# zjwfufu/FateAvatar

Hardware: AMD Instinct MI355X
Metric: render+backward frames/sec at 512^2, 100k Gaussians (higher is better)
Workload: dtype f32

## Files before the change

fateavatar_amd/csrc/fr_preprocess_bwd.hip:

```cpp
#include "fr_bind_math.hpp"

namespace fr {

__constant__ float bSH_C0 = 0.28209479177387814f;
__constant__ float bSH_C1 = 0.4886025119029199f;
__constant__ float bSH_C2[5] = {1.0925484305920792f, -1.0925484305920792f, 0.31539156525252005f,
                                -1.0925484305920792f, 0.5462742152960396f};
__constant__ float bSH_C3[7] = {-0.5900435899266435f, 2.890611442640554f, -0.4570457994644658f, 0.3731763325901154f,
                                -0.4570457994644658f, 1.445305721320277f,  -0.5900435899266435f};

struct PreBwdArgs {
    int P, D, M, W, H, raw;
    float tan_fovx, tan_fovy, focal_x, focal_y, scale_modifier;
    const float* means3D;
    const float* scales;
    const float* rotations;
    const float* shs;
    const float* cov3D_precomp;
    const float* view;
    const float* proj;
    const float* campos;
    const int* radii;
    GeomView g;
    fr_grads out;
    float* grad_accum;
    float* denom;
    float* overflow_out;
    const DeviceCounts* counts;
    uint32_t acc;
    int bound;
    BindArgs bind;
    BindGrads bg;
};

enum { G_MEANS2D = 0, G_COLORS, G_OPACITY, G_MEANS3D, G_COV3D, G_SH, G_SCALES, G_ROTATIONS };

__device__ __forceinline__ void put(float* p, float v, bool add) { *p = add ? *p + v : v; }

__device__ __forceinline__ void store3(float* p, size_t i, float a, float b, float c, bool add)
{
    if (!p) return;
    if (add) a += p[3 * i], b += p[3 * i + 1], c += p[3 * i + 2];
    p[3 * i] = a, p[3 * i + 1] = b, p[3 * i + 2] = c;
}

__host__ __device__ constexpr bool prebwd_rows_by16(int M3) { return M3 % 4 == 0 && M3 <= 48; }
__host__ __device__ constexpr int prebwd_row_stride(int M3)
{
    return prebwd_rows_by16(M3) ? (((M3 / 4) & 1) ? M3 : M3 + 4) : (M3 | 1);
}

struct PreBwdIn {
    int radius;
    float mean[3], q[4], sc[3], c3[6];
    float opacity;
    uint32_t cl;
    float dd[9];
    float4 r0, r1, r2;
    uint32_t overflow;
    float ga, dn;
    float old_m3[3], old_sc[3], old_q[4], old_op;
};

template <class T> using GlobalPtr = const __attribute__((address_space(1))) T*;
template <class T> __device__ __forceinline__ GlobalPtr<T> as_global(const T* p) { return (GlobalPtr<T>)p; }
typedef float PreBwdF4 __attribute__((ext_vector_type(4)));

__device__ __forceinline__ void preprocess_bwd_fetch(const PreBwdArgs& a, const int li, PreBwdIn& in)
{
    const size_t i = (size_t)li;
    const auto adds = [&](int k) { return ((a.acc >> k) & 1u) != 0u; };
    const int* radii_ = a.radii;
    const DeviceCounts* counts_ = a.counts;
    const float *accum_ = a.g.accum, *means3D_ = a.means3D, *scales_ = a.scales, *rotations_ = a.rotations, *cov3D_ = a.cov3D_precomp;
    const float *opacity_act_ = a.g.opacity_act, *dcolor_ddir_ = a.g.dcolor_ddir, *shs = a.shs;
    const uint8_t* clamped_ = a.g.clamped;
    const float *grad_accum_ = a.grad_accum, *denom_ = a.denom;
    asm volatile("" : "+s"(radii_), "+s"(counts_), "+s"(accum_), "+s"(means3D_), "+s"(scales_), "+s"(rotations_), "+s"(cov3D_),
                 "+s"(opacity_act_), "+s"(dcolor_ddir_), "+s"(shs), "+s"(clamped_), "+s"(grad_accum_), "+s"(denom_));
    const auto radii = as_global(radii_);
    const auto counts = as_global(counts_);
    const auto accum = as_global(accum_), means3D = as_global(means3D_), scales = as_global(scales_), rotations = as_global(rotations_);
    const auto cov3D = as_global(cov3D_), opacity_act = as_global(opacity_act_), dcolor_ddir = as_global(dcolor_ddir_);
    const auto clamped = as_global(clamped_);
    const auto grad_accum = as_global(grad_accum_), denom = as_global(denom_);
    in.radius = radii[li];
    in.overflow = counts->overflow;
    const GlobalPtr<PreBwdF4> row4 = (GlobalPtr<PreBwdF4>)(accum + i * kAccumStride);
    const PreBwdF4 r0 = row4[0], r1 = row4[1], r2 = row4[2];
    in.r0 = make_float4(r0.x, r0.y, r0.z, r0.w), in.r1 = make_float4(r1.x, r1.y, r1.z, r1.w), in.r2 = make_float4(r2.x, r2.y, r2.z, r2.w);
    for (int k = 0; k < 3; k++) in.mean[k] = means3D[3 * i + k];
    for (int k = 0; k < 4; k++) in.q[k] = 0.f;
    for (int k = 0; k < 3; k++) in.sc[k] = 0.f;
    for (int k = 0; k < 6; k++) in.c3[k] = 0.f;
    if (scales) {
        for (int k = 0; k < 4; k++) in.q[k] = rotations[4 * i + k];
        for (int k = 0; k < 3; k++) in.sc[k] = scales[3 * i + k];
    }
    if (cov3D)
        for (int k = 0; k < 6; k++) in.c3[k] = cov3D[6 * i + k];
    in.opacity = opacity_act[li];
    in.cl = 0u;
    for (int k = 0; k < 9; k++) in.dd[k] = 0.f;
    if (shs) {
        in.cl = clamped[li];
        for (int k = 0; k < 9; k++) in.dd[k] = dcolor_ddir[i * 9 + k];
    }
    in.ga = in.dn = 0.f;
    if (grad_accum) in.ga = grad_accum[i];
    if (denom) in.dn = denom[i];
    for (int k = 0; k < 3; k++) in.old_m3[k] = 0.f, in.old_sc[k] = 0.f;
    for (int k = 0; k < 4; k++) in.old_q[k] = 0.f;
    in.old_op = 0.f;
    if (a.acc) {
        if (adds(G_MEANS3D) && a.out.dL_dmeans3D)
            for (int k = 0; k < 3; k++) in.old_m3[k] = a.out.dL_dmeans3D[3 * i + k];
        if (adds(G_SCALES) && a.out.dL_dscales)
            for (int k = 0; k < 3; k++) in.old_sc[k] = a.out.dL_dscales[3 * i + k];
        if (adds(G_ROTATIONS) && a.out.dL_drotations)
            for (int k = 0; k < 4; k++) in.old_q[k] = a.out.dL_drotations[4 * i + k];
        if (adds(G_OPACITY) && a.out.dL_dopacity) in.old_op = a.out.dL_dopacity[i];
    }
}

template <bool PLANES>
__device__ __forceinline__ void preprocess_bwd_one(const PreBwdArgs& a, const CameraRegs& cam, const PreBwdIn& in,
                                                   const int idx, float* row, const bool by16)
{
    const size_t i = (size_t)idx;
    const int Mc = a.M;
    const int radius = in.radius;
    const auto adds = [&](int k) { return ((a.acc >> k) & 1u) != 0u; };
    if (!(radius > 0)) {
        if (row && by16) {
            float4* r4 = reinterpret_cast<float4*>(row);
            for (int k = 0; k < (Mc * 3) / 4; k++) r4[k] = make_float4(0.f, 0.f, 0.f, 0.f);
        } else if (row)
            for (int k = 0; k < Mc * 3; k++) row[k] = 0.f;
        if (!adds(G_MEANS2D)) store3(a.out.dL_dmeans2D, i, 0.f, 0.f, 0.f, false);
        if (!adds(G_COLORS)) store3(a.out.dL_dcolors, i, 0.f, 0.f, 0.f, false);
        if (a.out.dL_dopacity && !adds(G_OPACITY)) a.out.dL_dopacity[i] = 0.f;
        if (!adds(G_MEANS3D)) store3(a.out.dL_dmeans3D, i, 0.f, 0.f, 0.f, false);
        if (a.out.dL_dcov3D && !adds(G_COV3D))
            for (int k = 0; k < 6; k++) a.out.dL_dcov3D[6 * i + k] = 0.f;
        if (a.out.dL_dsh && !row && !adds(G_SH))
            for (int k = 0; k < Mc * 3; k++) a.out.dL_dsh[i * Mc * 3 + k] = 0.f;
        if (!adds(G_SCALES)) store3(a.out.dL_dscales, i, 0.f, 0.f, 0.f, false);
        if (a.out.dL_drotations && !adds(G_ROTATIONS))
            for (int k = 0; k < 4; k++) a.out.dL_drotations[4 * i + k] = 0.f;
        if (a.bound) bind_bwd_zero(idx, a.bg);
        return;
    }
    const float old_m3[3] = {in.old_m3[0], in.old_m3[1], in.old_m3[2]}, old_sc[3] = {in.old_sc[0], in.old_sc[1], in.old_sc[2]};
    const float old_q[4] = {in.old_q[0], in.old_q[1], in.old_q[2], in.old_q[3]}, old_op = in.old_op;
    float acc[12];
    {
        float4* row4 = reinterpret_cast<float4*>(a.g.accum + i * kAccumStride);
        const float4 r0 = in.r0, r1 = in.r1, r2 = in.r2;
        row4[0] = row4[1] = row4[2] = make_float4(0.f, 0.f, 0.f, 0.f);
        acc[0] = r0.x, acc[1] = r0.y, acc[2] = r0.z, acc[3] = r0.w, acc[4] = r1.x, acc[5] = r1.y, acc[6] = r1.z,
        acc[7] = r1.w, acc[8] = r2.x, acc[9] = r2.y, acc[10] = r2.z, acc[11] = r2.w;
    }
    const float3 mean = make_float3(in.mean[0], in.mean[1], in.mean[2]);
    const float* vm = cam.view;
    float q_r = 0.f, q_x = 0.f, q_y = 0.f, q_z = 0.f, rot_inv = 1.0f;
    float sc[3] = {0.f, 0.f, 0.f};
    float c3[6];
    if (a.scales) {
        q_r = in.q[0], q_x = in.q[1], q_y = in.q[2], q_z = in.q[3];
        sc[0] = in.sc[0], sc[1] = in.sc[1], sc[2] = in.sc[2];
        if (a.raw) {
            sc[0] = act_exp(sc[0]), sc[1] = act_exp(sc[1]), sc[2] = act_exp(sc[2]);
            rot_inv = act_rot_inv_norm(q_r, q_x, q_y, q_z);
            q_r *= rot_inv, q_x *= rot_inv, q_y *= rot_inv, q_z *= rot_inv;
        }
    }
    if (a.cov3D_precomp) {
        for (int k = 0; k < 6; k++) c3[k] = in.c3[k];
    } else {
        cov3d_from_scale_rot(sc[0], sc[1], sc[2], q_r, q_x, q_y, q_z, a.scale_modifier, c3);
    }

    float3 t = xform4x3(mean, vm);
    const float limx = 1.3f * a.tan_fovx, limy = 1.3f * a.tan_fovy;
    const float txtz = t.x / t.z, tytz = t.y / t.z;
    t.x = fminf(limx, fmaxf(-limx, txtz)) * t.z;
    t.y = fminf(limy, fmaxf(-limy, tytz)) * t.z;
    const float x_grad_mul = txtz < -limx || txtz > limx ? 0 : 1;
    const float y_grad_mul = tytz < -limy || tytz > limy ? 0 : 1;
    const float h_x = a.focal_x, h_y = a.focal_y;
    const float j00 = h_x / t.z, j02 = -(h_x * t.x) / (t.z * t.z);
    const float j11 = h_y / t.z, j12 = -(h_y * t.y) / (t.z * t.z);
    float T0[3], T1[3];
    for (int w = 0; w < 3; w++) {
        const float W0 = vm[4 * w], W1 = vm[4 * w + 1], W2 = vm[4 * w + 2];
        T0[w] = W0 * j00 + W1 * 0.0f + W2 * j02;
        T1[w] = W0 * 0.0f + W1 * j11 + W2 * j12;
    }
    const float V[3][3] = {{c3[0], c3[1], c3[2]}, {c3[1], c3[3], c3[4]}, {c3[2], c3[4], c3[5]}};
    float A0[3], A1[3];
    for (int c = 0; c < 3; c++) {
        A0[c] = T0[0] * V[0][c] + T0[1] * V[1][c] + T0[2] * V[2][c];
        A1[c] = T1[0] * V[0][c] + T1[1] * V[1][c] + T1[2] * V[2][c];
    }
    float ca = A0[0] * T0[0] + A0[1] * T0[1] + A0[2] * T0[2];
    const float cb = A1[0] * T0[0] + A1[1] * T0[1] + A1[2] * T0[2];
    float cc = A1[0] * T1[0] + A1[1] * T1[1] + A1[2] * T1[2];
    ca += 0.3f;
    cc += 0.3f;
    const float denom = ca * cc - cb * cb;
    const float det_inv = 1.f / denom;
    const float4 co = make_float4(cc * det_inv, -cb * det_inv, ca * det_inv, in.opacity);
    const float g2x = acc[ACC_MX] * (0.5f * a.W);
    const float g2y = acc[ACC_MY] * (0.5f * a.H);
    const float dcx = -0.5f * acc[ACC_CA], dcy = -0.5f * acc[ACC_CB], dcz = -0.5f * acc[ACC_CC];
    const float dop = (co.w != 0.f) ? acc[ACC_OP] / co.w : 0.f;
    float dcol[3] = {acc[ACC_R], acc[ACC_G], acc[ACC_B]};
    store3(a.out.dL_dmeans2D, i, g2x, g2y, 0.f, adds(G_MEANS2D));
    if (!in.overflow) {
        if (a.grad_accum) a.grad_accum[i] = in.ga + sqrtf(g2x * g2x + g2y * g2y);
        if (a.denom) a.denom[i] = in.dn + 1.0f;
    }
    store3(a.out.dL_dcolors, i, dcol[0], dcol[1], dcol[2], adds(G_COLORS));
    if (a.out.dL_dopacity) a.out.dL_dopacity[i] = old_op + (a.raw ? dop * co.w * (1.0f - co.w) : dop);

    float dL_da = 0, dL_db = 0, dL_dc = 0;
    const float denom2inv = 1.0f / ((denom * denom) + 0.0000001f);
    float dcov[6] = {0, 0, 0, 0, 0, 0};
    if (denom2inv != 0) {
        dL_da = denom2inv * (-cc * cc * dcx + 2 * cb * cc * dcy + (denom - ca * cc) * dcz);
        dL_dc = denom2inv * (-ca * ca * dcz + 2 * ca * cb * dcy + (denom - ca * cc) * dcx);
        dL_db = denom2inv * 2 * (cb * cc * dcx - (denom + 2 * cb * cb) * dcy + ca * cb * dcz);
        dcov[0] = (T0[0] * T0[0] * dL_da + T0[0] * T1[0] * dL_db + T1[0] * T1[0] * dL_dc);
        dcov[3] = (T0[1] * T0[1] * dL_da + T0[1] * T1[1] * dL_db + T1[1] * T1[1] * dL_dc);
        dcov[5] = (T0[2] * T0[2] * dL_da + T0[2] * T1[2] * dL_db + T1[2] * T1[2] * dL_dc);
        dcov[1] = 2 * T0[0] * T0[1] * dL_da + (T0[0] * T1[1] + T0[1] * T1[0]) * dL_db + 2 * T1[0] * T1[1] * dL_dc;
        dcov[2] = 2 * T0[0] * T0[2] * dL_da + (T0[0] * T1[2] + T0[2] * T1[0]) * dL_db + 2 * T1[0] * T1[2] * dL_dc;
        dcov[4] = 2 * T0[2] * T0[1] * dL_da + (T0[1] * T1[2] + T0[2] * T1[1]) * dL_db + 2 * T1[1] * T1[2] * dL_dc;
    }
    if (a.out.dL_dcov3D)
        for (int k = 0; k < 6; k++) put(a.out.dL_dcov3D + 6 * i + k, dcov[k], adds(G_COV3D));

    float dT0[3], dT1[3];
    for (int c = 0; c < 3; c++) {
        const float tv0 = T0[0] * V[c][0] + T0[1] * V[c][1] + T0[2] * V[c][2];
        const float tv1 = T1[0] * V[c][0] + T1[1] * V[c][1] + T1[2] * V[c][2];
        dT0[c] = 2 * tv0 * dL_da + tv1 * dL_db;
        dT1[c] = 2 * tv1 * dL_dc + tv0 * dL_db;
    }
    const float dL_dJ00 = vm[0] * dT0[0] + vm[4] * dT0[1] + vm[8] * dT0[2];
    const float dL_dJ02 = vm[2] * dT0[0] + vm[6] * dT0[1] + vm[10] * dT0[2];
    const float dL_dJ11 = vm[1] * dT1[0] + vm[5] * dT1[1] + vm[9] * dT1[2];
    const float dL_dJ12 = vm[2] * dT1[0] + vm[6] * dT1[1] + vm[10] * dT1[2];
    const float tz = 1.f / t.z, tz2 = tz * tz, tz3 = tz2 * tz;
    const float dL_dtx = x_grad_mul * -h_x * tz2 * dL_dJ02;
    const float dL_dty = y_grad_mul * -h_y * tz2 * dL_dJ12;
    const float dL_dtz = -h_x * tz2 * dL_dJ00 - h_y * tz2 * dL_dJ11 + (2 * h_x * t.x) * tz3 * dL_dJ02 + (2 * h_y * t.y) * tz3 * dL_dJ12;
    float dmx = vm[0] * dL_dtx + vm[1] * dL_dty + vm[2] * dL_dtz;
    float dmy = vm[4] * dL_dtx + vm[5] * dL_dty + vm[6] * dL_dtz;
    float dmz = vm[8] * dL_dtx + vm[9] * dL_dty + vm[10] * dL_dtz;

    {
        const float* proj = cam.proj;
        const float4 m_hom = xform4x4(mean, proj);
        const float m_w = 1.0f / (m_hom.w + 0.0000001f);
        const float mul1 = (proj[0] * mean.x + proj[4] * mean.y + proj[8] * mean.z + proj[12]) * m_w * m_w;
        const float mul2 = (proj[1] * mean.x + proj[5] * mean.y + proj[9] * mean.z + proj[13]) * m_w * m_w;
        const float px = (proj[0] * m_w - proj[3] * mul1) * g2x + (proj[1] * m_w - proj[3] * mul2) * g2y;
        const float py = (proj[4] * m_w - proj[7] * mul1) * g2x + (proj[5] * m_w - proj[7] * mul2) * g2y;
        const float pz = (proj[8] * m_w - proj[11] * mul1) * g2x + (proj[9] * m_w - proj[11] * mul2) * g2y;
        dmx += px, dmy += py, dmz += pz;
    }

    if (a.shs) {
        const float dox = mean.x - cam.campos[0], doy = mean.y - cam.campos[1], doz = mean.z - cam.campos[2];
        const float len = sqrtf(dox * dox + doy * doy + doz * doz);
        const float x = dox / len, y = doy / len, z = doz / len;
        const uint32_t cl = in.cl;
        float dRGB[3];
        for (int c = 0; c < 3; c++) dRGB[c] = dcol[c] * (((cl >> c) & 1) ? 0 : 1);
        const float* dd = in.dd;
        const float dRGBdx[3] = {dd[0], dd[1], dd[2]}, dRGBdy[3] = {dd[3], dd[4], dd[5]}, dRGBdz[3] = {dd[6], dd[7], dd[8]};
        const int deg = a.D;
        const int used = (deg + 1) * (deg + 1);
        auto write_row = [&](float* dsh, const bool dsh_adds) {
#define DSH(k, c, v_) put(dsh + (k) * 3 + (c), (v_), dsh_adds)
            for (int c = 0; c < 3; c++) {
                DSH(0, c, bSH_C0 * dRGB[c]);
                if (deg > 0) {
                    DSH(1, c, (-bSH_C1 * y) * dRGB[c]);
                    DSH(2, c, (bSH_C1 * z) * dRGB[c]);
                    DSH(3, c, (-bSH_C1 * x) * dRGB[c]);
                    if (deg > 1) {
                        const float xx = x * x, yy = y * y, zz = z * z;
                        const float xy = x * y, yz = y * z, xz = x * z;
                        DSH(4, c, (bSH_C2[0] * xy) * dRGB[c]);
                        DSH(5, c, (bSH_C2[1] * yz) * dRGB[c]);
                        DSH(6, c, (bSH_C2[2] * (2.f * zz - xx - yy)) * dRGB[c]);
                        DSH(7, c, (bSH_C2[3] * xz) * dRGB[c]);
                        DSH(8, c, (bSH_C2[4] * (xx - yy)) * dRGB[c]);
                        if (deg > 2) {
                            DSH(9, c, (bSH_C3[0] * y * (3.f * xx - yy)) * dRGB[c]);
                            DSH(10, c, (bSH_C3[1] * xy * z) * dRGB[c]);
                            DSH(11, c, (bSH_C3[2] * y * (4.f * zz - xx - yy)) * dRGB[c]);
                            DSH(12, c, (bSH_C3[3] * z * (2.f * zz - 3.f * xx - 3.f * yy)) * dRGB[c]);
                            DSH(13, c, (bSH_C3[4] * x * (4.f * zz - xx - yy)) * dRGB[c]);
                            DSH(14, c, (bSH_C3[5] * z * (xx - yy)) * dRGB[c]);
                            DSH(15, c, (bSH_C3[6] * x * (xx - 3.f * yy)) * dRGB[c]);
                        }
                    }
                }
            }
            if (!dsh_adds)
                for (int k = used; k < Mc; k++) dsh[k * 3] = 0.f, dsh[k * 3 + 1] = 0.f, dsh[k * 3 + 2] = 0.f;
#undef DSH
        };
        auto write_row_by16 = [&](float* dsh) {
            float f[16] = {0.f, 0.f, 0.f, 0.f, 0.f, 0.f, 0.f, 0.f, 0.f, 0.f, 0.f, 0.f, 0.f, 0.f, 0.f, 0.f};
            f[0] = bSH_C0;
            if (deg > 0) {
                f[1] = -bSH_C1 * y, f[2] = bSH_C1 * z, f[3] = -bSH_C1 * x;
                if (deg > 1) {
                    const float xx = x * x, yy = y * y, zz = z * z;
                    const float xy = x * y, yz = y * z, xz = x * z;
                    f[4] = bSH_C2[0] * xy, f[5] = bSH_C2[1] * yz, f[6] = bSH_C2[2] * (2.f * zz - xx - yy);
                    f[7] = bSH_C2[3] * xz, f[8] = bSH_C2[4] * (xx - yy);
                    if (deg > 2) {
                        f[9] = bSH_C3[0] * y * (3.f * xx - yy), f[10] = bSH_C3[1] * xy * z;
                        f[11] = bSH_C3[2] * y * (4.f * zz - xx - yy), f[12] = bSH_C3[3] * z * (2.f * zz - 3.f * xx - 3.f * yy);
                        f[13] = bSH_C3[4] * x * (4.f * zz - xx - yy), f[14] = bSH_C3[5] * z * (xx - yy);
                        f[15] = bSH_C3[6] * x * (xx - 3.f * yy);
                    }
                }
            }
            float4* d4 = reinterpret_cast<float4*>(dsh);
            const int pieces = (Mc * 3) / 4;
#pragma unroll
            for (int j = 0; j < 12; j++) {
                if (j >= pieces) break;
                float v[4];
#pragma unroll
                for (int t = 0; t < 4; t++) {
                    const int k = (4 * j + t) / 3, c = (4 * j + t) % 3;
                    v[t] = k < used ? f[k] * dRGB[c] : 0.f;
                }
                d4[j] = make_float4(v[0], v[1], v[2], v[3]);
            }
        };
        if (row && by16) write_row_by16(row);
        else if (row) write_row(row, false);
        else if (a.out.dL_dsh) write_row(a.out.dL_dsh + i * Mc * 3, adds(G_SH));
        const float ddx = dRGBdx[0] * dRGB[0] + dRGBdx[1] * dRGB[1] + dRGBdx[2] * dRGB[2];
        const float ddy = dRGBdy[0] * dRGB[0] + dRGBdy[1] * dRGB[1] + dRGBdy[2] * dRGB[2];
        const float ddz = dRGBdz[0] * dRGB[0] + dRGBdz[1] * dRGB[1] + dRGBdz[2] * dRGB[2];
        const float sum2 = dox * dox + doy * doy + doz * doz;
        const float invsum32 = 1.0f / sqrtf(sum2 * sum2 * sum2);
        dmx += ((+sum2 - dox * dox) * ddx - doy * dox * ddy - doz * dox * ddz) * invsum32;
        dmy += (-dox * doy * ddx + (sum2 - doy * doy) * ddy - doz * doy * ddz) * invsum32;
        dmz += (-dox * doz * ddx - doy * doz * ddy + (sum2 - doz * doz) * ddz) * invsum32;
    } else if (a.out.dL_dsh && !row && !adds(G_SH)) {
        for (int k = 0; k < Mc * 3; k++) a.out.dL_dsh[i * Mc * 3 + k] = 0.f;
    }
    if (PLANES) {
        const float dz = acc[ACC_Z];
        dmx += dz * vm[2], dmy += dz * vm[6], dmz += dz * vm[10];
    }
    store3(a.out.dL_dmeans3D, i, old_m3[0] + dmx, old_m3[1] + dmy, old_m3[2] + dmz, false);
    const float g_mean[3] = {dmx, dmy, dmz};
    float g_scl[3] = {0.f, 0.f, 0.f}, g_rot[4] = {0.f, 0.f, 0.f, 0.f};

    if (a.scales) {
        const float r = q_r, x = q_x, y = q_y, z = q_z;
        const float s[3] = {a.scale_modifier * sc[0], a.scale_modifier * sc[1], a.scale_modifier * sc[2]};
        const float Rc[3][3] = {{1.f - 2.f * (y * y + z * z), 2.f * (x * y - r * z), 2.f * (x * z + r * y)},
                                {2.f * (x * y + r * z), 1.f - 2.f * (x * x + z * z), 2.f * (y * z - r * x)},
                                {2.f * (x * z - r * y), 2.f * (y * z + r * x), 1.f - 2.f * (x * x + y * y)}};
        const float dS[3][3] = {{dcov[0], 0.5f * dcov[1], 0.5f * dcov[2]},
                                {0.5f * dcov[1], dcov[3], 0.5f * dcov[4]},
                                {0.5f * dcov[2], 0.5f * dcov[4], dcov[5]}};
        float dM[3][3];
        for (int c = 0; c < 3; c++)
            for (int w = 0; w < 3; w++)
                dM[c][w] = (s[w] * Rc[0][w] * 2.0f) * dS[c][0] + (s[w] * Rc[1][w] * 2.0f) * dS[c][1] + (s[w] * Rc[2][w] * 2.0f) * dS[c][2];
        float dMt[3][3];
        for (int c = 0; c < 3; c++)
            for (int w = 0; w < 3; w++) dMt[c][w] = dM[w][c];
        const float dsx = Rc[0][0] * dMt[0][0] + Rc[1][0] * dMt[0][1] + Rc[2][0] * dMt[0][2];
        const float dsy = Rc[0][1] * dMt[1][0] + Rc[1][1] * dMt[1][1] + Rc[2][1] * dMt[1][2];
        const float dsz = Rc[0][2] * dMt[2][0] + Rc[1][2] * dMt[2][1] + Rc[2][2] * dMt[2][2];
        g_scl[0] = a.raw ? dsx * sc[0] : dsx, g_scl[1] = a.raw ? dsy * sc[1] : dsy, g_scl[2] = a.raw ? dsz * sc[2] : dsz;
        store3(a.out.dL_dscales, i, old_sc[0] + g_scl[0], old_sc[1] + g_scl[1], old_sc[2] + g_scl[2], false);
        for (int w = 0; w < 3; w++) dMt[0][w] *= s[0], dMt[1][w] *= s[1], dMt[2][w] *= s[2];
#define Dm(c_, r_) dMt[c_][r_]
        if (a.out.dL_drotations || a.bound) {
            float dq[4];
            dq[0] = 2 * z * (Dm(0, 1) - Dm(1, 0)) + 2 * y * (Dm(2, 0) - Dm(0, 2)) + 2 * x * (Dm(1, 2) - Dm(2, 1));
            dq[1] = 2 * y * (Dm(1, 0) + Dm(0, 1)) + 2 * z * (Dm(2, 0) + Dm(0, 2)) + 2 * r * (Dm(1, 2) - Dm(2, 1)) - 4 * x * (Dm(2, 2) + Dm(1, 1));
            dq[2] = 2 * x * (Dm(1, 0) + Dm(0, 1)) + 2 * r * (Dm(2, 0) - Dm(0, 2)) + 2 * z * (Dm(1, 2) + Dm(2, 1)) - 4 * y * (Dm(2, 2) + Dm(0, 0));
            dq[3] = 2 * r * (Dm(0, 1) - Dm(1, 0)) + 2 * x * (Dm(2, 0) + Dm(0, 2)) + 2 * y * (Dm(1, 2) + Dm(2, 1)) - 4 * z * (Dm(1, 1) + Dm(0, 0));
            if (a.raw) {
                const float dot = r * dq[0] + x * dq[1] + y * dq[2] + z * dq[3];
                dq[0] = (dq[0] - r * dot) * rot_inv;
                dq[1] = (dq[1] - x * dot) * rot_inv;
                dq[2] = (dq[2] - y * dot) * rot_inv;
                dq[3] = (dq[3] - z * dot) * rot_inv;
            }
            if (a.out.dL_drotations)
                for (int k = 0; k < 4; k++) a.out.dL_drotations[4 * i + k] = old_q[k] + dq[k];
            for (int k = 0; k < 4; k++) g_rot[k] = dq[k];
        }
#undef Dm
    } else {
        if (!adds(G_SCALES)) store3(a.out.dL_dscales, i, 0.f, 0.f, 0.f, false);
        if (a.out.dL_drotations && !adds(G_ROTATIONS))
            for (int k = 0; k < 4; k++) a.out.dL_drotations[4 * i + k] = 0.f;
    }
    if (a.bound) bind_bwd(a.bind, idx, g_mean, g_rot, g_scl, a.bg);
}

template <bool ADD>
__device__ __forceinline__ void unstage_rows_t(float* __restrict__ dst, const float* src, int stride, int rows, int row_len, int lane)
{
    const int total = rows * row_len;
    const unsigned magic = (unsigned)((0x100000000ull + (unsigned)row_len - 1u) / (unsigned)row_len);
    constexpr int kBatch = ADD ? 6 : 1;
    for (int base = lane * 4; base < total; base += 64 * 4 * kBatch) {
        float4 o[kBatch];
        if (ADD) {
#pragma unroll
            for (int u = 0; u < kBatch; u++) {
                const int c = base + u * 64 * 4;
                o[u] = make_float4(0.f, 0.f, 0.f, 0.f);
                if (c + 3 < total) {
                    o[u] = *reinterpret_cast<const float4*>(dst + c);
                } else {
                    if (c < total) o[u].x = dst[c];
                    if (c + 1 < total) o[u].y = dst[c + 1];
                    if (c + 2 < total) o[u].z = dst[c + 2];
                }
            }
        }
#pragma unroll
        for (int u = 0; u < kBatch; u++) {
            const int c = base + u * 64 * 4;
            if (c >= total) break;
            float v[4];
#pragma unroll
            for (int k = 0; k < 4; k++) {
                const int e = c + k;
                const int r = (int)__umulhi((unsigned)e, magic);
                v[k] = (e < total) ? src[r * stride + (e - r * row_len)] : 0.f;
            }
            if (ADD) v[0] += o[u].x, v[1] += o[u].y, v[2] += o[u].z, v[3] += o[u].w;
            if (c + 3 < total) *reinterpret_cast<float4*>(dst + c) = make_float4(v[0], v[1], v[2], v[3]);
            else
                for (int k = 0; k < 4; k++)
                    if (c + k < total) dst[c + k] = v[k];
        }
    }
}
template <bool ADD>
__device__ __forceinline__ void unstage_rows_by16_t(float* __restrict__ dst, const float* src, int stride, int rows, int row_len, int lane)
{
    const int total = rows * row_len;
    const unsigned magic = (unsigned)((0x100000000ull + (unsigned)row_len - 1u) / (unsigned)row_len);
    constexpr int kBatch = ADD ? 6 : 1;
    for (int base = lane * 4; base < total; base += 64 * 4 * kBatch) {
        float4 o[kBatch];
        if (ADD) {
#pragma unroll
            for (int u = 0; u < kBatch; u++) {
                const int c = base + u * 64 * 4;
                o[u] = make_float4(0.f, 0.f, 0.f, 0.f);
                if (c < total) o[u] = *reinterpret_cast<const float4*>(dst + c);
            }
        }
#pragma unroll
        for (int u = 0; u < kBatch; u++) {
            const int c = base + u * 64 * 4;
            if (c >= total) break;
            const int r = (int)__umulhi((unsigned)c, magic);
            float4 v = *reinterpret_cast<const float4*>(src + r * stride + (c - r * row_len));
            if (ADD) v.x += o[u].x, v.y += o[u].y, v.z += o[u].z, v.w += o[u].w;
            *reinterpret_cast<float4*>(dst + c) = v;
        }
    }
}
__device__ __forceinline__ void unstage_rows(float* __restrict__ dst, const float* src, int stride, int rows, int row_len, int lane,
                                             bool add)
{
    if (prebwd_rows_by16(row_len)) {
        if (add) unstage_rows_by16_t<true>(dst, src, stride, rows, row_len, lane);
        else unstage_rows_by16_t<false>(dst, src, stride, rows, row_len, lane);
    } else {
        if (add) unstage_rows_t<true>(dst, src, stride, rows, row_len, lane);
        else unstage_rows_t<false>(dst, src, stride, rows, row_len, lane);
    }
}

#ifndef FR_PREBWD_WAVES
#define FR_PREBWD_WAVES 4
#endif
constexpr int kPreBwdWaves = FR_PREBWD_WAVES;

template <bool PLANES>
__device__ __forceinline__ void preprocess_bwd_body(const PreBwdArgs& a)
{
    extern __shared__ __attribute__((aligned(16))) float s_rows[];
    if ((int)(blockIdx.x * blockDim.x) >= a.P) return;
    const int idx = blockIdx.x * blockDim.x + threadIdx.x;
    const int lane = threadIdx.x & 63, wave = threadIdx.x >> 6;
    const int M3 = a.M * 3, stride = prebwd_row_stride(M3);
    const int wave_first = blockIdx.x * (64 * kPreBwdWaves) + wave * 64;
    const int rows = min(64, a.P - wave_first);
    const bool staged = a.shs != nullptr && a.out.dL_dsh != nullptr;
    float* w_rows = s_rows + (size_t)wave * 64 * stride;
    PreBwdIn in;
    preprocess_bwd_fetch(a, min(idx, a.P - 1), in);
    const float cam_x = camera_request(a.view, a.proj, a.campos, lane);
    asm volatile("" ::: "memory");
    const CameraRegs cam = camera_broadcast(cam_x);
    asm volatile("" : "+v"(in.cl), "+v"(in.ga), "+v"(in.dn), "+v"(in.opacity), "+v"(in.radius));
    if (a.overflow_out && blockIdx.x == 0 && threadIdx.x == 0) *a.overflow_out = in.overflow ? 1.0f : 0.0f;
    if (idx < a.P) preprocess_bwd_one<PLANES>(a, cam, in, idx, staged ? w_rows + lane * stride : nullptr, prebwd_rows_by16(M3));
    __syncthreads();
    if (staged && rows > 0) unstage_rows(a.out.dL_dsh + (size_t)wave_first * M3, w_rows, stride, rows, M3, lane, ((a.acc >> G_SH) & 1u) != 0u);
}

__global__ void __launch_bounds__(64 * kPreBwdWaves) k_preprocess_bwd(PreBwdArgs a) { preprocess_bwd_body<false>(a); }
__global__ void __launch_bounds__(64 * kPreBwdWaves) k_preprocess_bwd_batch(BatchOf<PreBwdArgs> b) { preprocess_bwd_body<false>(b.v[blockIdx.y]); }
__global__ void __launch_bounds__(64 * kPreBwdWaves) k_preprocess_bwd_planes(PreBwdArgs a) { preprocess_bwd_body<true>(a); }
__global__ void __launch_bounds__(64 * kPreBwdWaves) k_preprocess_bwd_planes_batch(BatchOf<PreBwdArgs> b) { preprocess_bwd_body<true>(b.v[blockIdx.y]); }

int launch_blend_backward(int n, const BackwardCall* calls, const GeomView* g, const ImageView* v, bool planes, hipStream_t s, bool debug);

int launch_backward(int n, const BackwardCall* calls, hipStream_t s)
{
    GeomView g[kMaxBatch];
    ImageView v[kMaxBatch];
    PreBwdArgs args[kMaxBatch];
    bool capturing = false, debug = false, planes = false;
    for (int k = 0; k < n; k++) capturing = note_capture(calls[k].h, s) || capturing;
    for (int k = 0; k < n; k++) {
        const fr_aux* aux = calls[k].prm->aux;
        planes = planes || ((calls[k].prm->flags & FR_FLAG_DEPTH_ALPHA) && aux && (aux->dL_ddepth || aux->dL_dalpha));
    }
    size_t lds = 0;
    uint32_t blocks = 0;
    const int wg = 64 * kPreBwdWaves;
    for (int k = 0; k < n; k++) {
        fr_handle_impl* h = calls[k].h;
        const fr_params& prm = *calls[k].prm;
        const fr_inputs& in = *calls[k].in;
        const int P = prm.P;
        g[k] = GeomView::make(calls[k].geometry, (size_t)P);
        if (!capturing && h->have_last_bwd && h->last_bwd_stream != s) FR_HIP(hipStreamWaitEvent(s, h->bwd_done, 0));
        {
            int rc0 = ensure_accum(h, (size_t)P, s);
            if (rc0) return rc0;
            g[k].accum = h->accum;
        }
        v[k] = ImageView::make(const_cast<void*>(calls[k].image), prm.W, prm.H);
        debug = debug || prm.debug != 0;
        PreBwdArgs& a = args[k];
        a.P = P, a.D = prm.D, a.M = prm.M, a.W = prm.W, a.H = prm.H;
        a.raw = (prm.flags & FR_FLAG_RAW_ACTIVATIONS) ? 1 : 0;
        a.tan_fovx = prm.tan_fovx, a.tan_fovy = prm.tan_fovy;
        a.focal_y = prm.H / (2.0f * prm.tan_fovy);
        a.focal_x = prm.W / (2.0f * prm.tan_fovx);
        a.scale_modifier = prm.scale_modifier;
        a.means3D = in.means3D, a.scales = in.scales, a.rotations = in.rotations, a.shs = in.shs;
        a.cov3D_precomp = in.cov3D_precomp, a.view = in.viewmatrix, a.proj = in.projmatrix, a.campos = in.campos;
        a.radii = calls[k].radii, a.g = g[k], a.out = *calls[k].grads;
        a.grad_accum = prm.aux ? prm.aux->grad_accum : nullptr;
        a.denom = prm.aux ? prm.aux->denom : nullptr;
        a.overflow_out = prm.aux ? prm.aux->overflow_out : nullptr;
        a.counts = v[k].counts;
        a.acc = ((uint32_t)prm.flags >> FR_FLAG_ACCUMULATE_SHIFT) & 0xFFu;
        a.bound = (prm.aux && prm.aux->binding) ? 1 : 0;
        if (a.bound) {
            a.bind = bind_args(*prm.aux->binding);
            a.bg = BindGrads{prm.aux->d_verts, prm.aux->d_offset, prm.aux->d_rotation, prm.aux->d_scaling, prm.aux->d_local_xyz};
        } else {
            a.bind = BindArgs{};
            a.bg = BindGrads{};
        }
        const size_t l = (in.shs && calls[k].grads->dL_dsh) ? (size_t)kPreBwdWaves * 64 * prebwd_row_stride(prm.M * 3) * sizeof(float) : 0;
        lds = l > lds ? l : lds;
        blocks = max(blocks, (uint32_t)((P + wg - 1) / wg));
    }
    int rc = launch_blend_backward(n, calls, g, v, planes, s, debug);
    if (rc) return rc;
    {
        StageScope sc(calls[0].h, ST_PREPROCESS_BWD, s);
        if (planes) launch_views(k_preprocess_bwd_planes, k_preprocess_bwd_planes_batch, n, args, blocks, (uint32_t)wg, lds, s);
        else launch_views(k_preprocess_bwd, k_preprocess_bwd_batch, n, args, blocks, (uint32_t)wg, lds, s);
    }
    FR_HIP(hipGetLastError());
    if (!capturing)
        for (int k = 0; k < n; k++) {
            fr_handle_impl* h = calls[k].h;
            FR_HIP(hipEventRecord(h->bwd_done, s));
            h->last_bwd_stream = s, h->have_last_bwd = true;
        }
    if (debug) FR_HIP(hipStreamSynchronize(s));
    return FR_OK;
}

}
```

Before: 23330.

## Stage SH gradient rows through LDS in 32-row chunks with wave-level fences

```diff
diff --git a/fateavatar_amd/csrc/fr_preprocess_bwd.hip b/fateavatar_amd/csrc/fr_preprocess_bwd.hip
--- a/fateavatar_amd/csrc/fr_preprocess_bwd.hip
+++ b/fateavatar_amd/csrc/fr_preprocess_bwd.hip
@@ -44,10 +44,71 @@
     p[3 * i] = a, p[3 * i + 1] = b, p[3 * i + 2] = c;
 }
 
+#ifndef FR_PREBWD_STAGE_ROWS
+#define FR_PREBWD_STAGE_ROWS 32
+#endif
+constexpr int kPreBwdStageRows = FR_PREBWD_STAGE_ROWS;
+static_assert(kPreBwdStageRows == 64 || kPreBwdStageRows == 32 || kPreBwdStageRows == 16, "FR_PREBWD_STAGE_ROWS: 64, 32 or 16");
+
 __host__ __device__ constexpr bool prebwd_rows_by16(int M3) { return M3 % 4 == 0 && M3 <= 48; }
 __host__ __device__ constexpr int prebwd_row_stride(int M3)
 {
     return prebwd_rows_by16(M3) ? (((M3 / 4) & 1) ? M3 : M3 + 4) : (M3 | 1);
+}
+__host__ __device__ constexpr int prebwd_block_rows(int M3) { return prebwd_rows_by16(M3) ? kPreBwdStageRows : 64; }
+
+struct PreBwdRow {
+    float x, y, z, dRGB[3];
+    bool visible;
+};
+
+__device__ __forceinline__ void write_row_by16(float* dsh, const PreBwdRow& r, const int deg, const int Mc)
+{
+    const float x = r.x, y = r.y, z = r.z;
+    const int used = (deg + 1) * (deg + 1);
+    float f[16] = {0.f, 0.f, 0.f, 0.f, 0.f, 0.f, 0.f, 0.f, 0.f, 0.f, 0.f, 0.f, 0.f, 0.f, 0.f, 0.f};
+    f[0] = bSH_C0;
+    if (deg > 0) {
+        f[1] = -bSH_C1 * y, f[2] = bSH_C1 * z, f[3] = -bSH_C1 * x;
+        if (deg > 1) {
+            const float xx = x * x, yy = y * y, zz = z * z;
+            const float xy = x * y, yz = y * z, xz = x * z;
+            f[4] = bSH_C2[0] * xy, f[5] = bSH_C2[1] * yz, f[6] = bSH_C2[2] * (2.f * zz - xx - yy);
+            f[7] = bSH_C2[3] * xz, f[8] = bSH_C2[4] * (xx - yy);
+            if (deg > 2) {
+                f[9] = bSH_C3[0] * y * (3.f * xx - yy), f[10] = bSH_C3[1] * xy * z;
+                f[11] = bSH_C3[2] * y * (4.f * zz - xx - yy), f[12] = bSH_C3[3] * z * (2.f * zz - 3.f * xx - 3.f * yy);
+                f[13] = bSH_C3[4] * x * (4.f * zz - xx - yy), f[14] = bSH_C3[5] * z * (xx - yy);
+                f[15] = bSH_C3[6] * x * (xx - 3.f * yy);
+            }
+        }
+    }
+    float4* d4 = reinterpret_cast<float4*>(dsh);
+    const int pieces = (Mc * 3) / 4;
+#pragma unroll
+    for (int j = 0; j < 12; j++) {
+        if (j < pieces) {
+            float v[4];
+#pragma unroll
+            for (int t = 0; t < 4; t++) {
+                const int k = (4 * j + t) / 3, c = (4 * j + t) % 3;
+                v[t] = k < used ? f[k] * r.dRGB[c] : 0.f;
+            }
+            d4[j] = make_float4(v[0], v[1], v[2], v[3]);
+        }
+    }
+}
+__device__ __forceinline__ void zero_row_by16(float* dsh, const int Mc)
+{
+    float4* d4 = reinterpret_cast<float4*>(dsh);
+    for (int k = 0; k < (Mc * 3) / 4; k++) d4[k] = make_float4(0.f, 0.f, 0.f, 0.f);
+}
+
+__device__ __forceinline__ void wave_lds_fence()
+{
+    __builtin_amdgcn_fence(__ATOMIC_RELEASE, "wavefront");
+    __builtin_amdgcn_wave_barrier();
+    __builtin_amdgcn_fence(__ATOMIC_ACQUIRE, "wavefront");
 }
 
 struct PreBwdIn {
@@ -125,17 +186,14 @@
 
 template <bool PLANES>
 __device__ __forceinline__ void preprocess_bwd_one(const PreBwdArgs& a, const CameraRegs& cam, const PreBwdIn& in,
-                                                   const int idx, float* row, const bool by16)
+                                                   const int idx, float* row, const bool defer, PreBwdRow& deferred)
 {
     const size_t i = (size_t)idx;
     const int Mc = a.M;
     const int radius = in.radius;
     const auto adds = [&](int k) { return ((a.acc >> k) & 1u) != 0u; };
     if (!(radius > 0)) {
-        if (row && by16) {
-            float4* r4 = reinterpret_cast<float4*>(row);
-            for (int k = 0; k < (Mc * 3) / 4; k++) r4[k] = make_float4(0.f, 0.f, 0.f, 0.f);
-        } else if (row)
+        if (row)
             for (int k = 0; k < Mc * 3; k++) row[k] = 0.f;
         if (!adds(G_MEANS2D)) store3(a.out.dL_dmeans2D, i, 0.f, 0.f, 0.f, false);
         if (!adds(G_COLORS)) store3(a.out.dL_dcolors, i, 0.f, 0.f, 0.f, false);
@@ -143,7 +201,7 @@
         if (!adds(G_MEANS3D)) store3(a.out.dL_dmeans3D, i, 0.f, 0.f, 0.f, false);
         if (a.out.dL_dcov3D && !adds(G_COV3D))
             for (int k = 0; k < 6; k++) a.out.dL_dcov3D[6 * i + k] = 0.f;
-        if (a.out.dL_dsh && !row && !adds(G_SH))
+        if (a.out.dL_dsh && !row && !defer && !adds(G_SH))
             for (int k = 0; k < Mc * 3; k++) a.out.dL_dsh[i * Mc * 3 + k] = 0.f;
         if (!adds(G_SCALES)) store3(a.out.dL_dscales, i, 0.f, 0.f, 0.f, false);
         if (a.out.dL_drotations && !adds(G_ROTATIONS))
@@ -315,40 +373,11 @@
                 for (int k = used; k < Mc; k++) dsh[k * 3] = 0.f, dsh[k * 3 + 1] = 0.f, dsh[k * 3 + 2] = 0.f;
 #undef DSH
         };
-        auto write_row_by16 = [&](float* dsh) {
-            float f[16] = {0.f, 0.f, 0.f, 0.f, 0.f, 0.f, 0.f, 0.f, 0.f, 0.f, 0.f, 0.f, 0.f, 0.f, 0.f, 0.f};
-            f[0] = bSH_C0;
-            if (deg > 0) {
-                f[1] = -bSH_C1 * y, f[2] = bSH_C1 * z, f[3] = -bSH_C1 * x;
-                if (deg > 1) {
-                    const float xx = x * x, yy = y * y, zz = z * z;
-                    const float xy = x * y, yz = y * z, xz = x * z;
-                    f[4] = bSH_C2[0] * xy, f[5] = bSH_C2[1] * yz, f[6] = bSH_C2[2] * (2.f * zz - xx - yy);
-                    f[7] = bSH_C2[3] * xz, f[8] = bSH_C2[4] * (xx - yy);
-                    if (deg > 2) {
-                        f[9] = bSH_C3[0] * y * (3.f * xx - yy), f[10] = bSH_C3[1] * xy * z;
-                        f[11] = bSH_C3[2] * y * (4.f * zz - xx - yy), f[12] = bSH_C3[3] * z * (2.f * zz - 3.f * xx - 3.f * yy);
-                        f[13] = bSH_C3[4] * x * (4.f * zz - xx - yy), f[14] = bSH_C3[5] * z * (xx - yy);
-                        f[15] = bSH_C3[6] * x * (xx - 3.f * yy);
-                    }
-                }
-            }
-            float4* d4 = reinterpret_cast<float4*>(dsh);
-            const int pieces = (Mc * 3) / 4;
-#pragma unroll
-            for (int j = 0; j < 12; j++) {
-                if (j >= pieces) break;
-                float v[4];
-#pragma unroll
-                for (int t = 0; t < 4; t++) {
-                    const int k = (4 * j + t) / 3, c = (4 * j + t) % 3;
-                    v[t] = k < used ? f[k] * dRGB[c] : 0.f;
-                }
-                d4[j] = make_float4(v[0], v[1], v[2], v[3]);
-            }
-        };
-        if (row && by16) write_row_by16(row);
-        else if (row) write_row(row, false);
+        if (defer) {
+            deferred.x = x, deferred.y = y, deferred.z = z;
+            deferred.dRGB[0] = dRGB[0], deferred.dRGB[1] = dRGB[1], deferred.dRGB[2] = dRGB[2];
+            deferred.visible = true;
+        } else if (row) write_row(row, false);
         else if (a.out.dL_dsh) write_row(a.out.dL_dsh + i * Mc * 3, adds(G_SH));
         const float ddx = dRGBdx[0] * dRGB[0] + dRGBdx[1] * dRGB[1] + dRGBdx[2] * dRGB[2];
         const float ddy = dRGBdy[0] * dRGB[0] + dRGBdy[1] * dRGB[1] + dRGBdy[2] * dRGB[2];
@@ -358,7 +387,7 @@
         dmx += ((+sum2 - dox * dox) * ddx - doy * dox * ddy - doz * dox * ddz) * invsum32;
         dmy += (-dox * doy * ddx + (sum2 - doy * doy) * ddy - doz * doy * ddz) * invsum32;
         dmz += (-dox * doz * ddx - doy * doz * ddy + (sum2 - doz * doz) * ddz) * invsum32;
-    } else if (a.out.dL_dsh && !row && !adds(G_SH)) {
+    } else if (a.out.dL_dsh && !row && !defer && !adds(G_SH)) {
         for (int k = 0; k < Mc * 3; k++) a.out.dL_dsh[i * Mc * 3 + k] = 0.f;
     }
     if (PLANES) {
@@ -486,17 +515,6 @@
         }
     }
 }
-__device__ __forceinline__ void unstage_rows(float* __restrict__ dst, const float* src, int stride, int rows, int row_len, int lane,
-                                             bool add)
-{
-    if (prebwd_rows_by16(row_len)) {
-        if (add) unstage_rows_by16_t<true>(dst, src, stride, rows, row_len, lane);
-        else unstage_rows_by16_t<false>(dst, src, stride, rows, row_len, lane);
-    } else {
-        if (add) unstage_rows_t<true>(dst, src, stride, rows, row_len, lane);
-        else unstage_rows_t<false>(dst, src, stride, rows, row_len, lane);
-    }
-}
 
 #ifndef FR_PREBWD_WAVES
 #define FR_PREBWD_WAVES 4
@@ -514,7 +532,8 @@
     const int wave_first = blockIdx.x * (64 * kPreBwdWaves) + wave * 64;
     const int rows = min(64, a.P - wave_first);
     const bool staged = a.shs != nullptr && a.out.dL_dsh != nullptr;
-    float* w_rows = s_rows + (size_t)wave * 64 * stride;
+    const bool by16 = prebwd_rows_by16(M3);
+    float* w_rows = s_rows + (size_t)wave * prebwd_block_rows(M3) * stride;
     PreBwdIn in;
     preprocess_bwd_fetch(a, min(idx, a.P - 1), in);
     const float cam_x = camera_request(a.view, a.proj, a.campos, lane);
@@ -522,9 +541,34 @@
     const CameraRegs cam = camera_broadcast(cam_x);
     asm volatile("" : "+v"(in.cl), "+v"(in.ga), "+v"(in.dn), "+v"(in.opacity), "+v"(in.radius));
     if (a.overflow_out && blockIdx.x == 0 && threadIdx.x == 0) *a.overflow_out = in.overflow ? 1.0f : 0.0f;
-    if (idx < a.P) preprocess_bwd_one<PLANES>(a, cam, in, idx, staged ? w_rows + lane * stride : nullptr, prebwd_rows_by16(M3));
-    __syncthreads();
-    if (staged && rows > 0) unstage_rows(a.out.dL_dsh + (size_t)wave_first * M3, w_rows, stride, rows, M3, lane, ((a.acc >> G_SH) & 1u) != 0u);
+    PreBwdRow mine;
+    mine.x = mine.y = mine.z = mine.dRGB[0] = mine.dRGB[1] = mine.dRGB[2] = 0.f, mine.visible = false;
+    if (idx < a.P)
+        preprocess_bwd_one<PLANES>(a, cam, in, idx, staged && !by16 ? w_rows + lane * stride : nullptr, staged && by16, mine);
+    if (!staged || rows <= 0) return;
+    float* dst = a.out.dL_dsh + (size_t)wave_first * M3;
+    const bool add = ((a.acc >> G_SH) & 1u) != 0u;
+    if (!by16) {
+        wave_lds_fence();
+        if (add) unstage_rows_t<true>(dst, w_rows, stride, rows, M3, lane);
+        else unstage_rows_t<false>(dst, w_rows, stride, rows, M3, lane);
+        return;
+    }
+    constexpr int R = kPreBwdStageRows;
+#pragma unroll
+    for (int first = 0; first < 64; first += R) {
+        if (first >= rows) break;
+        if (lane >= first && lane < first + R) {
+            float* row = w_rows + (lane - first) * stride;
+            if (mine.visible) write_row_by16(row, mine, a.D, a.M);
+            else zero_row_by16(row, a.M);
+        }
+        wave_lds_fence();
+        const int n = min(R, rows - first);
+        if (add) unstage_rows_by16_t<true>(dst + (size_t)first * M3, w_rows, stride, n, M3, lane);
+        else unstage_rows_by16_t<false>(dst + (size_t)first * M3, w_rows, stride, n, M3, lane);
+        wave_lds_fence();
+    }
 }
 
 __global__ void __launch_bounds__(64 * kPreBwdWaves) k_preprocess_bwd(PreBwdArgs a) { preprocess_bwd_body<false>(a); }
@@ -585,7 +629,7 @@
             a.bind = BindArgs{};
             a.bg = BindGrads{};
         }
-        const size_t l = (in.shs && calls[k].grads->dL_dsh) ? (size_t)kPreBwdWaves * 64 * prebwd_row_stride(prm.M * 3) * sizeof(float) : 0;
+        const size_t l = (in.shs && calls[k].grads->dL_dsh) ? (size_t)kPreBwdWaves * prebwd_block_rows(prm.M * 3) * prebwd_row_stride(prm.M * 3) * sizeof(float) : 0;
         lds = l > lds ? l : lds;
         blocks = max(blocks, (uint32_t)((P + wg - 1) / wg));
     }
```

New measurement: 23810 (median of 6 runs). 1.02x the previous value.
